# microsoft/M3P

Hardware: AMD Instinct MI355X
Metric: pre-train samples/sec (whole node), 12L/768d seq=128+36 (higher is better)
Workload: dtype bf16; 1 GPU; cfg2: 12L/768d/12h, 36 regions + 128 tokens, V=250002, 19 MLM targets/seq + ITM BCE, dropout 0.10, adam_inverse_sqrt + clip 5; per_gpu_batch=256, global_batch=256, seq_len=164, parallelism=dp1, prewarm_steps=36

## Files before the change

### m3p_amd/csrc/embed.hip

```cpp
#include "common.hpp"
#include <hip/amd_detail/amd_hip_unsafe_atomics.h>

namespace {

constexpr int EMB_BWD_BLOCKS = 512;

constexpr float kEps = 1e-12f;

template <int NI>
__device__ __forceinline__ void row_ln(const f32x4 (&v)[NI], int nchunk, int lane, float inv_d, float& mu, float& rs) {
  float s = 0.f;
#pragma unroll
  for (int i = 0; i < NI; ++i) s += (v[i][0] + v[i][1]) + (v[i][2] + v[i][3]);
  mu = wave_sum(s) * inv_d;
  float q = 0.f;
#pragma unroll
  for (int i = 0; i < NI; ++i) {
    if (lane + 64 * i < nchunk) {
      const f32x4 t = v[i] - mu;
      q += (t[0] * t[0] + t[1] * t[1]) + (t[2] * t[2] + t[3] * t[3]);
    }
  }
  rs = 1.0f / sqrtf(wave_sum(q) * inv_d + kEps);
}

struct EmbedFwdArgs {
  const int64_t* tok;
  const bf16* emb;
  const float* pos;
  const bf16* img_proj;
  const float* loc;
  const float* w_loc;
  const float* b_loc;
  const float* g_img; const float* be_img;
  const float* g_emb; const float* be_emb;
  const int32_t* totlen;
  bf16* h;
  bf16* z;
  float* mean_emb; float* rstd_emb;
  bf16* e;
  float* mean_img; float* rstd_img;
  int B, T, R, d;
  uint32_t seed_img, seed_emb, thresh24; float inv_keep;
  bf16* img_rows; int img_mode;
};

template <int NI>
__global__ __launch_bounds__(256) void embed_fwd_kernel(EmbedFwdArgs a) {
  const int lane = threadIdx.x & 63;
  const int wave = (blockIdx.x * blockDim.x + threadIdx.x) >> 6;
  const int nwaves = (gridDim.x * blockDim.x) >> 6;
  const int S = a.R + a.T, d = a.d, nchunk = d >> 2;
  const float inv_d = 1.0f / (float)d;
  for (int m = wave; m < a.B * S; m += nwaves) {
    const int b = m / S, s = m - b * S;
    const float mk = (a.img_mode == 1 || s < a.totlen[b]) ? 1.f : 0.f;
    f32x4 v[NI];
    if (s < a.R && a.img_mode == 2) {
#pragma unroll
      for (int i = 0; i < NI; ++i) {
        const int c = lane + 64 * i;
        v[i] = f32x4{0.f, 0.f, 0.f, 0.f};
        if (c < nchunk) v[i] = Vec4<bf16>::load(a.img_rows + ((size_t)b * a.R + s) * d + 4 * c);
      }
    } else if (s < a.R) {
      const int ri = s * a.B + b;
      float lc[5];
#pragma unroll
      for (int k = 0; k < 5; ++k) lc[k] = a.loc[(size_t)ri * 5 + k];
#pragma unroll
      for (int i = 0; i < NI; ++i) {
        const int c = lane + 64 * i;
        v[i] = f32x4{0.f, 0.f, 0.f, 0.f};
        if (c < nchunk) {
          f32x4 t = Vec4<bf16>::load(a.img_proj + (size_t)ri * d + 4 * c) + Vec4<float>::load(a.b_loc + 4 * c);
#pragma unroll
          for (int j = 0; j < 4; ++j) {
            const float* w = a.w_loc + (size_t)(4 * c + j) * 5;
            t[j] += w[0] * lc[0] + w[1] * lc[1] + w[2] * lc[2] + w[3] * lc[3] + w[4] * lc[4];
          }
          t = round_bf16(t);
          Vec4<bf16>::store(a.e + (size_t)ri * d + 4 * c, t);
          v[i] = t;
        }
      }
      float mu, rs;
      row_ln<NI>(v, nchunk, lane, inv_d, mu, rs);
      if (lane == 0) { a.mean_img[ri] = mu; a.rstd_img[ri] = rs; }
#pragma unroll
      for (int i = 0; i < NI; ++i) {
        const int c = lane + 64 * i;
        if (c < nchunk) {
          f32x4 o = (v[i] - mu) * rs * Vec4<float>::load(a.g_img + 4 * c) + Vec4<float>::load(a.be_img + 4 * c);
          if (a.thresh24) {
            const uint32_t base = (uint32_t)ri * (uint32_t)d + 4u * c;
            { bool kp[4]; m3p_keep_even<4>(base, a.seed_img, a.thresh24, kp);
#pragma unroll
          for (int j = 0; j < 4; ++j) o[j] = kp[j] ? o[j] * a.inv_keep : 0.f; }
          }
          v[i] = o;
          if (a.img_mode == 1) Vec4<bf16>::store(a.img_rows + ((size_t)b * a.R + s) * d + 4 * c, o);
        }
      }
      if (a.img_mode == 1) continue;
    } else {
      const int64_t id = a.tok[(size_t)(s - a.R) * a.B + b];
#pragma unroll
      for (int i = 0; i < NI; ++i) {
        const int c = lane + 64 * i;
        v[i] = f32x4{0.f, 0.f, 0.f, 0.f};
        if (c < nchunk) v[i] = Vec4<bf16>::load(a.emb + (size_t)id * d + 4 * c);
      }
    }
#pragma unroll
    for (int i = 0; i < NI; ++i) {
      const int c = lane + 64 * i;
      if (c < nchunk) {
        const f32x4 t = round_bf16((v[i] + Vec4<float>::load(a.pos + (size_t)s * d + 4 * c)) * mk);
        Vec4<bf16>::store(a.z + (size_t)m * d + 4 * c, t);
        v[i] = t;
      }
    }
    float mu, rs;
    row_ln<NI>(v, nchunk, lane, inv_d, mu, rs);
    if (lane == 0) { a.mean_emb[m] = mu; a.rstd_emb[m] = rs; }
#pragma unroll
    for (int i = 0; i < NI; ++i) {
      const int c = lane + 64 * i;
      if (c < nchunk) {
        f32x4 o = (v[i] - mu) * rs * Vec4<float>::load(a.g_emb + 4 * c) + Vec4<float>::load(a.be_emb + 4 * c);
        if (a.thresh24) {
          const uint32_t base = (uint32_t)m * (uint32_t)d + 4u * c;
          { bool kp[4]; m3p_keep_even<4>(base, a.seed_emb, a.thresh24, kp);
#pragma unroll
          for (int j = 0; j < 4; ++j) o[j] = kp[j] ? o[j] * a.inv_keep : 0.f; }
        }
        Vec4<bf16>::store(a.h + (size_t)m * d + 4 * c, o);
      }
    }
  }
}

struct EmbedBwdArgs {
  const bf16* dh;
  const bf16* z; const float* mean_emb; const float* rstd_emb; const float* g_emb;
  const bf16* e; const float* mean_img; const float* rstd_img; const float* g_img;
  const int64_t* tok; const int32_t* totlen; const float* loc;
  bf16* dz;
  bf16* de;
  float* d_g_emb; float* d_be_emb; float* d_pos;
  float* d_emb;
  bf16* d_tok_rows;
  float* d_g_img; float* d_be_img; float* d_b_img; float* d_b_loc; float* d_w_loc;
  int B, T, R, d, pad_index, bsplit;
  uint32_t seed_img, seed_emb, thresh24; float inv_keep;
};

template <int NI>
__device__ __forceinline__ void block_reduce_atomic(float (*red)[NI * 256], const f32x4 (&acc)[NI], float* out, int d,
                                                    int lane, int wib) {
#pragma unroll
  for (int i = 0; i < NI; ++i)
#pragma unroll
    for (int j = 0; j < 4; ++j) red[wib][4 * (lane + 64 * i) + j] = acc[i][j];
  __syncthreads();
  for (int c = threadIdx.x; c < d; c += blockDim.x)
    unsafeAtomicAdd(out + c, (red[0][c] + red[1][c]) + (red[2][c] + red[3][c]));
  __syncthreads();
}

template <int NI>
__global__ __launch_bounds__(256) void embed_bwd_rows_kernel(EmbedBwdArgs a) {
  __shared__ float red[4][NI * 256];
  const int lane = threadIdx.x & 63, wib = threadIdx.x >> 6;
  const int S = a.R + a.T, d = a.d, nchunk = d >> 2;
  const float inv_d = 1.0f / (float)d;
  const int s = blockIdx.x / a.bsplit, part = blockIdx.x - s * a.bsplit;
  f32x4 g[NI], acc_g[NI], acc_b[NI], acc_p[NI];
#pragma unroll
// ... 55 lines not shown
        if (c < nchunk) {
          f32x4 o = *reinterpret_cast<const f32x4*>(&red[wib][4 * c]);
          if (!live) o = f32x4{0.f, 0.f, 0.f, 0.f};
          Vec4<bf16>::store(dr + 4 * c, o);
        }
      }
    } else if (s >= a.R && id != a.pad_index && mk != 0.f) {
      float* de = a.d_emb + (size_t)id * d;
#pragma unroll
      for (int k = 0; k < 4 * NI; ++k) {
        const int e = lane + 64 * k;
        if (e < d) unsafeAtomicAdd(de + e, red[wib][e]);
      }
    }
  }
  __syncthreads();
  block_reduce_atomic<NI>(red, acc_g, a.d_g_emb, d, lane, wib);
  block_reduce_atomic<NI>(red, acc_b, a.d_be_emb, d, lane, wib);
  block_reduce_atomic<NI>(red, acc_p, a.d_pos + (size_t)s * d, d, lane, wib);
}

template <int NI>
__global__ __launch_bounds__(256) void embed_bwd_img_kernel(EmbedBwdArgs a) {
  __shared__ float red[4][NI * 256];
  const int lane = threadIdx.x & 63, wib = threadIdx.x >> 6;
  const int S = a.R + a.T, d = a.d, nchunk = d >> 2;
  const float inv_d = 1.0f / (float)d;
  const int r = blockIdx.x / a.bsplit, part = blockIdx.x - r * a.bsplit;
  f32x4 g[NI], acc_g[NI], acc_b[NI], acc_e[NI], acc_w[5][NI];
#pragma unroll
  for (int i = 0; i < NI; ++i) {
    const int c = lane + 64 * i;
    g[i] = f32x4{0.f, 0.f, 0.f, 0.f};
    if (c < nchunk) g[i] = Vec4<float>::load(a.g_img + 4 * c);
    acc_g[i] = acc_b[i] = acc_e[i] = f32x4{0.f, 0.f, 0.f, 0.f};
#pragma unroll
    for (int k = 0; k < 5; ++k) acc_w[k][i] = f32x4{0.f, 0.f, 0.f, 0.f};
  }
  for (int b = part * 4 + wib; b < a.B; b += 4 * a.bsplit) {
    const size_t m = (size_t)b * S + r;
    const size_t ri = (size_t)r * a.B + b;
    const float mu = a.mean_img[ri], rs = a.rstd_img[ri];
    float lc[5];
#pragma unroll
    for (int k = 0; k < 5; ++k) lc[k] = a.loc[ri * 5 + k];
    f32x4 dy[NI], xh[NI];
    float s1 = 0.f, s2 = 0.f;
#pragma unroll
    for (int i = 0; i < NI; ++i) {
      const int c = lane + 64 * i;
      dy[i] = xh[i] = f32x4{0.f, 0.f, 0.f, 0.f};
      if (c < nchunk) {
        dy[i] = Vec4<bf16>::load(a.dz + m * d + 4 * c);
        if (a.thresh24) {
          const uint32_t base = (uint32_t)ri * (uint32_t)d + 4u * c;
          { bool kp[4]; m3p_keep_even<4>(base, a.seed_img, a.thresh24, kp);
#pragma unroll
          for (int j = 0; j < 4; ++j) dy[i][j] = kp[j] ? dy[i][j] * a.inv_keep : 0.f; }
        }
        xh[i] = (Vec4<bf16>::load(a.e + ri * d + 4 * c) - mu) * rs;
        const f32x4 gd = dy[i] * g[i];
        s1 += (gd[0] + gd[1]) + (gd[2] + gd[3]);
        const f32x4 gx = gd * xh[i];
        s2 += (gx[0] + gx[1]) + (gx[2] + gx[3]);
        acc_g[i] += dy[i] * xh[i];
        acc_b[i] += dy[i];
      }
    }
    const float c1 = wave_sum(s1) * inv_d, c2 = wave_sum(s2) * inv_d;
#pragma unroll
    for (int i = 0; i < NI; ++i) {
      const int c = lane + 64 * i;
      if (c < nchunk) {
        const f32x4 ob = round_bf16((dy[i] * g[i] - c1 - xh[i] * c2) * rs);
        Vec4<bf16>::store(a.de + ri * d + 4 * c, ob);
        acc_e[i] += ob;
#pragma unroll
        for (int k = 0; k < 5; ++k) acc_w[k][i] += ob * lc[k];
      }
    }
  }
  block_reduce_atomic<NI>(red, acc_g, a.d_g_img, d, lane, wib);
  block_reduce_atomic<NI>(red, acc_b, a.d_be_img, d, lane, wib);
#pragma unroll
  for (int i = 0; i < NI; ++i)
#pragma unroll
    for (int j = 0; j < 4; ++j) red[wib][4 * (lane + 64 * i) + j] = acc_e[i][j];
  __syncthreads();
  for (int c = threadIdx.x; c < d; c += blockDim.x) {
    const float v = (red[0][c] + red[1][c]) + (red[2][c] + red[3][c]);
    unsafeAtomicAdd(a.d_b_img + c, v);
    unsafeAtomicAdd(a.d_b_loc + c, v);
  }
  __syncthreads();
#pragma unroll
  for (int k = 0; k < 5; ++k) {
#pragma unroll
    for (int i = 0; i < NI; ++i)
#pragma unroll
      for (int j = 0; j < 4; ++j) red[wib][4 * (lane + 64 * i) + j] = acc_w[k][i][j];
    __syncthreads();
    for (int c = threadIdx.x; c < d; c += blockDim.x)
      unsafeAtomicAdd(a.d_w_loc + (size_t)c * 5 + k, (red[0][c] + red[1][c]) + (red[2][c] + red[3][c]));
    __syncthreads();
  }
}

__global__ __launch_bounds__(256) void cast_f32_bf16_kernel(const float* __restrict__ src, bf16* __restrict__ dst, size_t n4) {
  for (size_t i = (size_t)blockIdx.x * blockDim.x + threadIdx.x; i < n4; i += (size_t)gridDim.x * blockDim.x)
    Vec4<bf16>::store(dst + 4 * i, Vec4<float>::load(src + 4 * i));
}

inline int ni_of(int d) { return (d + 255) / 256; }

int launch_embed_fwd(const EmbedFwdArgs& a, void* stream);
}

extern "C" {

int m3p_cast_f32_bf16(const float* src, void* dst, long long n, void* stream) {
  if (n <= 0 || (n % 4) != 0 || ((uintptr_t)src & 15) || ((uintptr_t)dst & 7)) return M3P_EINVAL;
  const size_t n4 = (size_t)n / 4;
  const int blocks = (int)((n4 + 255) / 256 < 4096 ? (n4 + 255) / 256 : 4096);
  hipLaunchKernelGGL(cast_f32_bf16_kernel, dim3(blocks), dim3(256), 0, (hipStream_t)stream, src, (bf16*)dst, n4);
  M3P_CHECK_LAUNCH();
  return M3P_OK;
}
// ... 9 lines not shown
  EmbedFwdArgs a = {tok, (const bf16*)emb_bf16, pos, (const bf16*)img_proj, loc, w_loc, b_loc, g_img, be_img, g_emb, be_emb,
                    totlen, (bf16*)h, (bf16*)z, mean_emb, rstd_emb, (bf16*)e, mean_img, rstd_img, B, T, R, d,
                    seed_img, seed_emb, thresh24, inv_keep, (bf16*)const_cast<void*>(img_rows), img_rows ? 2 : 0};
  return launch_embed_fwd(a, stream);
}

int m3p_embed_image_rows_fwd(const void* img_proj, const float* loc, const float* w_loc, const float* b_loc,
                             const float* g_img, const float* be_img, void* e, float* mean_img, float* rstd_img,
                             void* img_rows, int B, int R, int d, uint32_t seed_img, uint32_t thresh24, float inv_keep,
                             void* stream) {
  if (B <= 0 || R <= 0 || d <= 0 || (d % 4) != 0 || d > 1024 || !img_rows || ((uintptr_t)img_rows & 7)) return M3P_EINVAL;
  EmbedFwdArgs a = {nullptr, nullptr, nullptr, (const bf16*)img_proj, loc, w_loc, b_loc, g_img, be_img, nullptr, nullptr,
                    nullptr, nullptr, nullptr, nullptr, nullptr, (bf16*)e, mean_img, rstd_img, B, 0, R, d,
                    seed_img, 0u, thresh24, inv_keep, (bf16*)img_rows, 1};
  return launch_embed_fwd(a, stream);
}

}

namespace {
int launch_embed_fwd(const EmbedFwdArgs& a, void* stream) {
  const int B = a.B, T = a.T, R = a.R, d = a.d;
  const int rows = B * (R + T);
  const int blocks = (rows + 3) / 4 < 4096 ? (rows + 3) / 4 : 4096;
  hipStream_t st = (hipStream_t)stream;
  switch (ni_of(d)) {
    case 1: hipLaunchKernelGGL(embed_fwd_kernel<1>, dim3(blocks), dim3(256), 0, st, a); break;
    case 2: hipLaunchKernelGGL(embed_fwd_kernel<2>, dim3(blocks), dim3(256), 0, st, a); break;
    case 3: hipLaunchKernelGGL(embed_fwd_kernel<3>, dim3(blocks), dim3(256), 0, st, a); break;
    default: hipLaunchKernelGGL(embed_fwd_kernel<4>, dim3(blocks), dim3(256), 0, st, a); break;
  }
  M3P_CHECK_LAUNCH();
  return M3P_OK;
}
}

extern "C" {

int m3p_embed_assemble_bwd(const void* dh, const void* z, const float* mean_emb, const float* rstd_emb,
                           const float* g_emb, const void* e, const float* mean_img, const float* rstd_img,
                           const float* g_img, const int64_t* tok, const int32_t* totlen, const float* loc,
                           void* dz_scratch, void* de, float* d_g_emb, float* d_be_emb, float* d_pos, float* d_emb,
                           void* d_tok_rows, float* d_g_img, float* d_be_img, float* d_b_img, float* d_b_loc, float* d_w_loc,
                           int B, int T, int R, int d, int pad_index, uint32_t seed_img, uint32_t seed_emb,
                           uint32_t thresh24, float inv_keep, int phase, void* stream) {
  if (B <= 0 || T < 0 || R < 0 || d <= 0 || (d % 4) != 0 || d > 1024 || phase < 0 || phase > 2) return M3P_EINVAL;
  int bsplit = 1;
  while (bsplit < 16 && (R + T) * bsplit < EMB_BWD_BLOCKS && B / (4 * bsplit) >= 8) bsplit *= 2;
  EmbedBwdArgs a = {(const bf16*)dh, (const bf16*)z, mean_emb, rstd_emb, g_emb, (const bf16*)e, mean_img, rstd_img, g_img,
                    tok, totlen, loc, (bf16*)dz_scratch, (bf16*)de, d_g_emb, d_be_emb, d_pos, d_emb,
                    (bf16*)d_tok_rows, d_g_img, d_be_img, d_b_img, d_b_loc, d_w_loc, B, T, R, d, pad_index, bsplit,
                    seed_img, seed_emb, thresh24, inv_keep};
  hipStream_t st = (hipStream_t)stream;
  const int S = R + T;
#define M3P_EMB_BWD(NI)                                                                              \
  do {                                                                                               \
    if (phase != 2) hipLaunchKernelGGL(embed_bwd_rows_kernel<NI>, dim3(S* bsplit), dim3(256), 0, st, a);             \
    if (R > 0 && phase != 1) hipLaunchKernelGGL(embed_bwd_img_kernel<NI>, dim3(R* bsplit), dim3(256), 0, st, a);   \
  } while (0)
  switch (ni_of(d)) {
    case 1: M3P_EMB_BWD(1); break;
    case 2: M3P_EMB_BWD(2); break;
    case 3: M3P_EMB_BWD(3); break;
    default: M3P_EMB_BWD(4); break;
  }
#undef M3P_EMB_BWD
  M3P_CHECK_LAUNCH();
  return M3P_OK;
}

}
```

### m3p_amd/csrc/glue.hip

```cpp
#include "common.hpp"

namespace {

__global__ __launch_bounds__(256)
void seq_masks_kernel(const long long* __restrict__ len_a, const long long* __restrict__ len_b, int B, int S,
                      int* __restrict__ totlen, uint8_t* __restrict__ rowmask) {
  const int b = blockIdx.x;
  const int n = (int)(len_a[b] + (len_b ? len_b[b] : 0));
  if (threadIdx.x == 0) totlen[b] = n;
  for (int s = threadIdx.x; s < S; s += blockDim.x) rowmask[(size_t)b * S + s] = (s < n) ? 1 : 0;
}

__global__ __launch_bounds__(1024)
void mask_to_rows_kernel(const uint8_t* __restrict__ mask, int n_mask, int inner, long long s0, long long s1,
                         long long soff, int d, int* __restrict__ rows, int n_rows) {
  __shared__ int wsum[16];
  __shared__ int total_sh;
  const int tid = threadIdx.x, lane = tid & 63, w = tid >> 6;
  const int per = (n_mask + 1023) / 1024;
  const int lo = min(tid * per, n_mask), hi = min(lo + per, n_mask);
  int cnt = 0;
  for (int i = lo; i < hi; ++i) cnt += mask[i] ? 1 : 0;
  int inc = cnt;
#pragma unroll
  for (int o = 1; o < 64; o <<= 1) {
    const int v = __shfl_up(inc, o, 64);
    if (lane >= o) inc += v;
  }
  if (lane == 63) wsum[w] = inc;
  __syncthreads();
  if (tid == 0) {
    int run = 0;
    for (int i = 0; i < 16; ++i) { const int v = wsum[i]; wsum[i] = run; run += v; }
    total_sh = run;
  }
  __syncthreads();
  int pos = wsum[w] + inc - cnt;
  for (int i = lo; i < hi; ++i) {
    if (mask[i]) {
      if (pos < n_rows) {
        const int t = i / inner, b = i - t * inner;
        rows[pos] = (int)((soff + t * s0 + b * s1) / d);
      }
      ++pos;
    }
  }
  for (int k = total_sh + tid; k < n_rows; k += 1024) rows[k] = 0;
}

__global__ __launch_bounds__(256)
void cast_rows_kernel(const float* __restrict__ in, long long s0, long long s1, int n1, int cols,
                      bf16* __restrict__ out, long long nrows) {
  const int cpr = cols >> 2;
  const long long total = nrows * cpr;
  for (long long i = (long long)blockIdx.x * blockDim.x + threadIdx.x; i < total; i += (long long)gridDim.x * blockDim.x) {
    const long long row = i / cpr;
    const int c = (int)(i - row * cpr) * 4;
    const long long i0 = row / n1, i1 = row - i0 * n1;
    const f32x4 v = *reinterpret_cast<const f32x4*>(in + i0 * s0 + i1 * s1 + c);
    *reinterpret_cast<bf16x4*>(out + row * cols + c) = bf16x4{(bf16)v[0], (bf16)v[1], (bf16)v[2], (bf16)v[3]};
  }
}

template <typename TI>
__global__ __launch_bounds__(256)
void scale_to_bf16_kernel(const TI* __restrict__ in, const float* __restrict__ g, bf16* __restrict__ out, long long n4) {
  const float s = g[0];
  for (long long i = (long long)blockIdx.x * blockDim.x + threadIdx.x; i < n4; i += (long long)gridDim.x * blockDim.x) {
    f32x4 v = Vec4<TI>::load(in + 4 * i);
    v *= s;
    Vec4<bf16>::store(out + 4 * i, v);
  }
}

__global__ __launch_bounds__(256)
void axpy_dev_kernel(float* __restrict__ dst, const float* __restrict__ src, const float* __restrict__ g, long long n) {
  const float s = g[0];
  for (long long i = (long long)blockIdx.x * blockDim.x + threadIdx.x; i < n; i += (long long)gridDim.x * blockDim.x)
    dst[i] += s * src[i];
}

__device__ __forceinline__ float softplus_f(float x) {
  return fmaxf(x, 0.f) + log1pf(__expf(-fabsf(x)));
// ... 40 lines not shown

int grid_for(long long work, int per_block) {
  long long g = (work + per_block - 1) / per_block;
  return (int)(g < 1 ? 1 : (g > 2048 ? 2048 : g));
}

}

extern "C" {

int m3p_seq_masks(const int64_t* lengths, const int64_t* lengths_b, int B, int S, int32_t* totlen, uint8_t* rowmask,
                  void* stream) {
  if (B <= 0 || S <= 0 || !lengths || !totlen || !rowmask) return M3P_EINVAL;
  hipLaunchKernelGGL(seq_masks_kernel, dim3(B), dim3(256), 0, (hipStream_t)stream, (const long long*)lengths,
                     (const long long*)lengths_b, B, S, totlen, rowmask);
  M3P_CHECK_LAUNCH();
  return M3P_OK;
}

int m3p_mask_to_rows(const uint8_t* mask, int n_mask, int inner, long long s0, long long s1, long long soff, int d,
                     int32_t* rows, int n_rows, void* stream) {
  if (n_mask <= 0 || inner <= 0 || d <= 0 || n_rows < 0 || !mask || (n_rows && !rows)) return M3P_EINVAL;
  if (n_rows == 0) return M3P_OK;
  hipLaunchKernelGGL(mask_to_rows_kernel, dim3(1), dim3(1024), 0, (hipStream_t)stream, mask, n_mask, inner, s0, s1, soff, d,
                     rows, n_rows);
  M3P_CHECK_LAUNCH();
  return M3P_OK;
}

int m3p_cast_rows_f32_bf16(const float* in, long long s0, long long s1, int n0, int n1, int cols, void* out, void* stream) {
  if (n0 <= 0 || n1 <= 0 || cols <= 0 || (cols & 3) || (s0 & 3) || (s1 & 3) || ((uintptr_t)in & 15) || ((uintptr_t)out & 7))
    return M3P_EINVAL;
  const long long nrows = (long long)n0 * n1;
  hipLaunchKernelGGL(cast_rows_kernel, dim3(grid_for(nrows * (cols >> 2), 1024)), dim3(256), 0, (hipStream_t)stream, in, s0, s1,
                     n1, cols, (bf16*)out, nrows);
  M3P_CHECK_LAUNCH();
  return M3P_OK;
}

int m3p_scale_bf16_dev(const void* in, int in_is_f32, const float* g, void* out, long long n, void* stream) {
  if (n <= 0 || (n & 3) || !g || ((uintptr_t)in & (in_is_f32 ? 15 : 7)) || ((uintptr_t)out & 7)) return M3P_EINVAL;
  const int grid = grid_for(n >> 2, 1024);
  if (in_is_f32)
    hipLaunchKernelGGL(scale_to_bf16_kernel<float>, dim3(grid), dim3(256), 0, (hipStream_t)stream, (const float*)in, g, (bf16*)out, n >> 2);
  else
    hipLaunchKernelGGL(scale_to_bf16_kernel<bf16>, dim3(grid), dim3(256), 0, (hipStream_t)stream, (const bf16*)in, g, (bf16*)out, n >> 2);
  M3P_CHECK_LAUNCH();
  return M3P_OK;
}

int m3p_axpy_dev_f32(float* dst, const float* src, const float* g, long long n, void* stream) {
  if (n <= 0 || !dst || !src || !g) return M3P_EINVAL;
  hipLaunchKernelGGL(axpy_dev_kernel, dim3(grid_for(n, 1024)), dim3(256), 0, (hipStream_t)stream, dst, src, g, n);
  M3P_CHECK_LAUNCH();
  return M3P_OK;
}

int m3p_itm_loss_fwd_bwd(const float* scores, const int64_t* pos, int n_groups, int sample_n, float w_ce, float w_bce,
// ... 10 lines not shown
```

### m3p_amd/csrc/heads.hip

```cpp
#include "common.hpp"
#include <hip/amd_detail/amd_hip_unsafe_atomics.h>

namespace {

__global__ __launch_bounds__(256) void gather_rows_kernel(const bf16* __restrict__ src, const int32_t* __restrict__ idx,
                                                          bf16* __restrict__ dst, int n, int d) {
  const int nchunk = d >> 2;
  const size_t total = (size_t)n * nchunk;
  for (size_t i = (size_t)blockIdx.x * blockDim.x + threadIdx.x; i < total; i += (size_t)gridDim.x * blockDim.x) {
    const int r = (int)(i / nchunk), c = (int)(i - (size_t)r * nchunk);
    *reinterpret_cast<bf16x4*>(dst + (size_t)r * d + 4 * c) =
        *reinterpret_cast<const bf16x4*>(src + (size_t)idx[r] * d + 4 * c);
  }
}
__global__ __launch_bounds__(256) void place_rows_kernel(const bf16* __restrict__ src, const int32_t* __restrict__ inv,
                                                         bf16* __restrict__ dst, int rows, int d, int n, uint32_t fill2) {
  typedef unsigned int u32x4 __attribute__((ext_vector_type(4)));
  const int nchunk = d >> 3;
  const size_t total = (size_t)rows * nchunk;
  const u32x4 fv = u32x4{fill2, fill2, fill2, fill2};
  for (size_t i = (size_t)blockIdx.x * blockDim.x + threadIdx.x; i < total; i += (size_t)gridDim.x * blockDim.x) {
    const int r = (int)(i / nchunk), c = (int)(i - (size_t)r * nchunk);
    const int j = inv[r];
    u32x4 v = fv;
// ... 209 lines not shown
      lb[u] = row_lse[r] * kLog2e;
      tc[u] = (int)(target[r] - col0);
    }
#pragma unroll
    for (int u = 0; u < U; ++u) {
      if (rb + u < r1) {
        bf16x8 g;
#pragma unroll
        for (int j = 0; j < 8; ++j) {
          float q = (col0 + j < V) ? __builtin_amdgcn_exp2f(__builtin_fmaf((float)v[u][j], kLog2e, -lb[u])) : 0.f;
          if (j == tc[u]) q -= 1.f;
          g[j] = (bf16)(q * gscale);
          cs[j] += (float)g[j];
        }
        *reinterpret_cast<bf16x8*>(logits + (size_t)(rb + u) * ld + col0) = g;
      }
    }
  }
  float* out = part + (size_t)blockIdx.y * ld + col0;
  *reinterpret_cast<f32x4*>(out) = f32x4{cs[0], cs[1], cs[2], cs[3]};
  *reinterpret_cast<f32x4*>(out + 4) = f32x4{cs[4], cs[5], cs[6], cs[7]};
}

__global__ __launch_bounds__(256) void ce_colsum_reduce_kernel(const float* __restrict__ part, int ld, int n_groups, float* __restrict__ out) {
  const int c = (blockIdx.x * 256 + threadIdx.x) * 4;
  if (c >= ld) return;
  const int per = (n_groups + gridDim.y - 1) / gridDim.y;
  const int g0 = blockIdx.y * per, g1 = min(n_groups, g0 + per);
  f32x4 acc = {0.f, 0.f, 0.f, 0.f};
  for (int g = g0; g < g1; ++g) acc += *reinterpret_cast<const f32x4*>(part + (size_t)g * ld + c);
#pragma unroll
  for (int j = 0; j < 4; ++j) unsafeAtomicAdd(out + c + j, acc[j]);
}

__global__ __launch_bounds__(256) void colsum_kernel(const bf16* __restrict__ x, int ld, int n, int ncols,
                                                     float* __restrict__ out, const float* __restrict__ scale_ptr) {
  const int c4 = blockIdx.x * blockDim.x + threadIdx.x;
  if (4 * c4 >= ncols) return;
  const int rows_per = (n + gridDim.y - 1) / gridDim.y;
  const int r0 = blockIdx.y * rows_per, r1 = min(n, r0 + rows_per);
  f32x4 acc = {0.f, 0.f, 0.f, 0.f};
  for (int r = r0; r < r1; ++r) acc += Vec4<bf16>::load(x + (size_t)r * ld + 4 * c4);
  const float sc = scale_ptr ? *scale_ptr : 1.f;
#pragma unroll
  for (int j = 0; j < 4; ++j)
    if (4 * c4 + j < ncols) unsafeAtomicAdd(out + 4 * c4 + j, acc[j] * sc);
}

}

extern "C" {

size_t m3p_ce_colsum_workspace_bytes(int ld, int n_rows) {
  return (size_t)((n_rows + CE_RB - 1) / CE_RB) * (size_t)ld * sizeof(float);
}
// ... 107 lines not shown
```

### m3p_amd/csrc/itm.hip

```cpp
#include "common.hpp"

namespace {

__global__ __launch_bounds__(256) void itm_score_fwd_kernel(const bf16* __restrict__ pre, const float* __restrict__ w2,
                                                            const float* __restrict__ b2, float* __restrict__ pooled,
                                                            float* __restrict__ scores, int d) {
  __shared__ float red[4];
  const int b = blockIdx.x, tid = threadIdx.x, lane = tid & 63, wid = tid >> 6;
  float s = 0.f;
  for (int j = tid; j < d; j += 256) {
    const float p = tanhf((float)pre[(size_t)b * d + j]);
    pooled[(size_t)b * d + j] = p;
    s += w2[j] * p;
  }
  s = wave_sum(s);
  if (lane == 0) red[wid] = s;
  __syncthreads();
  if (tid == 0) scores[b] = red[0] + red[1] + red[2] + red[3] + b2[0];
}

__global__ __launch_bounds__(256) void itm_score_bwd_rows_kernel(const float* __restrict__ dscores, const float* __restrict__ pooled,
                                                                 const float* __restrict__ w2, bf16* __restrict__ dpre16,
                                                                 bf16* __restrict__ dpreT16, int ldt, int d) {
  const int b = blockIdx.x;
  const float ds = dscores[b];
  for (int j = threadIdx.x; j < d; j += 256) {
    const float p = pooled[(size_t)b * d + j];
    const bf16 g = (bf16)(ds * w2[j] * (1.f - p * p));
    dpre16[(size_t)b * d + j] = g;
    dpreT16[(size_t)j * ldt + b] = g;
  }
}

__global__ __launch_bounds__(256) void itm_score_bwd_cols_kernel(const float* __restrict__ dscores, const float* __restrict__ pooled,
                                                                 const float* __restrict__ w2, float* __restrict__ db1,
                                                                 float* __restrict__ dw2, float* __restrict__ db2, int B, int d) {
  __shared__ float s1[4][64], s2[4][64], s3[4];
  const int jl = threadIdx.x & 63, bg = threadIdx.x >> 6;
  const int j = blockIdx.x * 64 + jl;
  float a1 = 0.f, a2 = 0.f, a3 = 0.f;
  if (j < d) {
    const float w = w2[j];
    for (int b = bg; b < B; b += 4) {
      const float ds = dscores[b], p = pooled[(size_t)b * d + j];
      a1 += ds * w * (1.f - p * p);
      a2 += ds * p;
      if (jl == 0) a3 += ds;
    }
  }
  s1[bg][jl] = a1; s2[bg][jl] = a2;
  if (jl == 0) s3[bg] = a3;
  __syncthreads();
  if (bg == 0 && j < d) {
    db1[j] += (s1[0][jl] + s1[1][jl]) + (s1[2][jl] + s1[3][jl]);
    dw2[j] += (s2[0][jl] + s2[1][jl]) + (s2[2][jl] + s2[3][jl]);
  }
  if (blockIdx.x == 0 && threadIdx.x == 0) db2[0] += (s3[0] + s3[1]) + (s3[2] + s3[3]);
}

}

extern "C" {

int m3p_itm_score_fwd(const void* pre, const float* w2, const float* b2, float* pooled, float* scores, int B, int d,
                      void* stream) {
  if (B <= 0 || d <= 0) return M3P_EINVAL;
  hipLaunchKernelGGL(itm_score_fwd_kernel, dim3(B), dim3(256), 0, (hipStream_t)stream, (const bf16*)pre, w2, b2, pooled,
                     scores, d);
  M3P_CHECK_LAUNCH();
  return M3P_OK;
}

int m3p_itm_score_bwd(const float* dscores, const float* pooled, const float* w2, void* dpre16, void* dpreT16, int ldt,
                      float* db1, float* dw2, float* db2, int B, int d, void* stream) {
  if (B <= 0 || d <= 0 || ldt < B) return M3P_EINVAL;
  hipLaunchKernelGGL(itm_score_bwd_rows_kernel, dim3(B), dim3(256), 0, (hipStream_t)stream, dscores, pooled, w2,
                     (bf16*)dpre16, (bf16*)dpreT16, ldt, d);
  M3P_CHECK_LAUNCH();
  hipLaunchKernelGGL(itm_score_bwd_cols_kernel, dim3((d + 63) / 64), dim3(256), 0, (hipStream_t)stream, dscores, pooled, w2,
                     db1, dw2, db2, B, d);
  M3P_CHECK_LAUNCH();
  return M3P_OK;
}

}
```

Baseline: 7847 sequences/s.

## Prefetch rows in embedding kernels and vectorize small glue reduction kernels

The embedding forward and image-backward kernels now issue the next row's loads before computing the current row (software prefetch), and the forward kernel stages w_loc transposed in LDS. Image-backward reductions are folded in two shared-memory stages with their own block split. Separately, mask_to_rows counts bits with 16-byte vector loads, cast_rows gains an 8-wide nontemporal path, the CE column-sum reduce is unrolled with coalesced atomics, and the ITM column kernel uses 1024 threads. These target memory latency and launch inefficiency in small kernels, at the cost of extra registers and LDS per block.

```diff
diff --git a/m3p_amd/csrc/embed.hip b/m3p_amd/csrc/embed.hip
--- a/m3p_amd/csrc/embed.hip
+++ b/m3p_amd/csrc/embed.hip
@@ -4,6 +4,8 @@
 namespace {
 
 constexpr int EMB_BWD_BLOCKS = 512;
+constexpr int EMB_BWD_IMG_BLOCKS = 256;
+constexpr int EMB_FWD_BLOCKS = 1536;
 
 constexpr float kEps = 1e-12f;
 
@@ -46,39 +48,83 @@
 };
 
 template <int NI>
+struct FwdRow {
+  bf16x4 raw[NI];
+  float lc[5];
+  int tl;
+};
+
+__device__ __forceinline__ int64_t embed_fwd_token(const EmbedFwdArgs& a, int m) {
+  const int S = a.R + a.T, b = m / S, s = m - b * S;
+  return s >= a.R ? a.tok[(size_t)(s - a.R) * a.B + b] : 0;
+}
+
+template <int NI>
+__device__ __forceinline__ void embed_fwd_request(const EmbedFwdArgs& a, int m, int64_t id, int lane, FwdRow<NI>& r) {
+  const int S = a.R + a.T, d = a.d, nchunk = d >> 2;
+  const int b = m / S, s = m - b * S;
+  r.tl = a.img_mode == 1 ? 0 : a.totlen[b];
+  const bf16* src;
+  if (s >= a.R) {
+    src = a.emb + (size_t)id * d;
+  } else if (a.img_mode == 2) {
+    src = a.img_rows + ((size_t)b * a.R + s) * d;
+  } else {
+    const int ri = s * a.B + b;
+    src = a.img_proj + (size_t)ri * d;
+#pragma unroll
+    for (int k = 0; k < 5; ++k) r.lc[k] = a.loc[(size_t)ri * 5 + k];
+  }
+#pragma unroll
+  for (int i = 0; i < NI; ++i) {
+    const int c = lane + 64 * i;
+    r.raw[i] = bf16x4{(bf16)0.f, (bf16)0.f, (bf16)0.f, (bf16)0.f};
+    if (c < nchunk) r.raw[i] = *reinterpret_cast<const bf16x4*>(src + 4 * c);
+  }
+}
+
+__device__ __forceinline__ f32x4 widen(bf16x4 v) { return f32x4{(float)v[0], (float)v[1], (float)v[2], (float)v[3]}; }
+
+template <int NI>
 __global__ __launch_bounds__(256) void embed_fwd_kernel(EmbedFwdArgs a) {
+  __shared__ __attribute__((aligned(16))) float wl[5][NI * 256];
   const int lane = threadIdx.x & 63;
   const int wave = (blockIdx.x * blockDim.x + threadIdx.x) >> 6;
   const int nwaves = (gridDim.x * blockDim.x) >> 6;
-  const int S = a.R + a.T, d = a.d, nchunk = d >> 2;
+  const int S = a.R + a.T, d = a.d, nchunk = d >> 2, rows = a.B * S;
   const float inv_d = 1.0f / (float)d;
-  for (int m = wave; m < a.B * S; m += nwaves) {
+  if (a.R > 0 && a.img_mode != 2) {
+    for (int i = threadIdx.x; i < 5 * d; i += 256) {
+      const int c = i / 5;
+      wl[i - 5 * c][c] = a.w_loc[i];
+    }
+    __syncthreads();
+  }
+  if (wave >= rows) return;
+  FwdRow<NI> nx;
+  embed_fwd_request<NI>(a, wave, embed_fwd_token(a, wave), lane, nx);
+  int64_t idn = wave + nwaves < rows ? embed_fwd_token(a, wave + nwaves) : 0;
+  for (int m = wave; m < rows; m += nwaves) {
     const int b = m / S, s = m - b * S;
-    const float mk = (a.img_mode == 1 || s < a.totlen[b]) ? 1.f : 0.f;
+    const FwdRow<NI> cu = nx;
+    if (m + nwaves < rows) {
+      embed_fwd_request<NI>(a, m + nwaves, idn, lane, nx);
+      if (m + 2 * nwaves < rows) idn = embed_fwd_token(a, m + 2 * nwaves);
+    }
+    const float mk = (a.img_mode == 1 || s < cu.tl) ? 1.f : 0.f;
     f32x4 v[NI];
-    if (s < a.R && a.img_mode == 2) {
+#pragma unroll
+    for (int i = 0; i < NI; ++i) v[i] = widen(cu.raw[i]);
+    if (s < a.R && a.img_mode != 2) {
+      const int ri = s * a.B + b;
 #pragma unroll
       for (int i = 0; i < NI; ++i) {
         const int c = lane + 64 * i;
-        v[i] = f32x4{0.f, 0.f, 0.f, 0.f};
-        if (c < nchunk) v[i] = Vec4<bf16>::load(a.img_rows + ((size_t)b * a.R + s) * d + 4 * c);
-      }
-    } else if (s < a.R) {
-      const int ri = s * a.B + b;
-      float lc[5];
-#pragma unroll
-      for (int k = 0; k < 5; ++k) lc[k] = a.loc[(size_t)ri * 5 + k];
-#pragma unroll
-      for (int i = 0; i < NI; ++i) {
-        const int c = lane + 64 * i;
-        v[i] = f32x4{0.f, 0.f, 0.f, 0.f};
         if (c < nchunk) {
-          f32x4 t = Vec4<bf16>::load(a.img_proj + (size_t)ri * d + 4 * c) + Vec4<float>::load(a.b_loc + 4 * c);
-#pragma unroll
-          for (int j = 0; j < 4; ++j) {
-            const float* w = a.w_loc + (size_t)(4 * c + j) * 5;
-            t[j] += w[0] * lc[0] + w[1] * lc[1] + w[2] * lc[2] + w[3] * lc[3] + w[4] * lc[4];
-          }
+          f32x4 t = v[i] + Vec4<float>::load(a.b_loc + 4 * c);
+          t += Vec4<float>::load(&wl[0][4 * c]) * cu.lc[0] + Vec4<float>::load(&wl[1][4 * c]) * cu.lc[1] +
+               Vec4<float>::load(&wl[2][4 * c]) * cu.lc[2] + Vec4<float>::load(&wl[3][4 * c]) * cu.lc[3] +
+               Vec4<float>::load(&wl[4][4 * c]) * cu.lc[4];
           t = round_bf16(t);
           Vec4<bf16>::store(a.e + (size_t)ri * d + 4 * c, t);
           v[i] = t;
@@ -103,14 +149,6 @@
         }
       }
       if (a.img_mode == 1) continue;
-    } else {
-      const int64_t id = a.tok[(size_t)(s - a.R) * a.B + b];
-#pragma unroll
-      for (int i = 0; i < NI; ++i) {
-        const int c = lane + 64 * i;
-        v[i] = f32x4{0.f, 0.f, 0.f, 0.f};
-        if (c < nchunk) v[i] = Vec4<bf16>::load(a.emb + (size_t)id * d + 4 * c);
-      }
     }
 #pragma unroll
     for (int i = 0; i < NI; ++i) {
@@ -152,9 +190,37 @@
   float* d_emb;
   bf16* d_tok_rows;
   float* d_g_img; float* d_be_img; float* d_b_img; float* d_b_loc; float* d_w_loc;
-  int B, T, R, d, pad_index, bsplit;
+  int B, T, R, d, pad_index, bsplit, bsplit_img;
   uint32_t seed_img, seed_emb, thresh24; float inv_keep;
 };
+
+template <int NI>
+__device__ __forceinline__ float* fold_at(float* red, int half, int q, int nq) { return red + (size_t)(half * nq + q) * (NI * 256); }
+
+template <int NI, int NQ>
+__device__ __forceinline__ void block_fold(float* red, f32x4 (&acc)[NQ][NI], int lane, int wib) {
+  if (wib >= 2) {
+#pragma unroll
+    for (int q = 0; q < NQ; ++q)
+#pragma unroll
+      for (int i = 0; i < NI; ++i) Vec4<float>::store(fold_at<NI>(red, wib - 2, q, NQ) + 4 * (lane + 64 * i), acc[q][i]);
+  }
+  __syncthreads();
+  if (wib < 2) {
+#pragma unroll
+    for (int q = 0; q < NQ; ++q)
+#pragma unroll
+      for (int i = 0; i < NI; ++i) acc[q][i] += Vec4<float>::load(fold_at<NI>(red, wib, q, NQ) + 4 * (lane + 64 * i));
+  }
+  __syncthreads();
+  if (wib < 2) {
+#pragma unroll
+    for (int q = 0; q < NQ; ++q)
+#pragma unroll
+      for (int i = 0; i < NI; ++i) Vec4<float>::store(fold_at<NI>(red, wib, q, NQ) + 4 * (lane + 64 * i), acc[q][i]);
+  }
+  __syncthreads();
+}
 
 template <int NI>
 __device__ __forceinline__ void block_reduce_atomic(float (*red)[NI * 256], const f32x4 (&acc)[NI], float* out, int d,
@@ -256,28 +322,44 @@
 
 template <int NI>
 __global__ __launch_bounds__(256) void embed_bwd_img_kernel(EmbedBwdArgs a) {
-  __shared__ float red[4][NI * 256];
+  __shared__ __attribute__((aligned(16))) float red[10 * NI * 256];
   const int lane = threadIdx.x & 63, wib = threadIdx.x >> 6;
   const int S = a.R + a.T, d = a.d, nchunk = d >> 2;
   const float inv_d = 1.0f / (float)d;
-  const int r = blockIdx.x / a.bsplit, part = blockIdx.x - r * a.bsplit;
-  f32x4 g[NI], acc_g[NI], acc_b[NI], acc_e[NI], acc_w[5][NI];
+  const int r = blockIdx.x / a.bsplit_img, part = blockIdx.x - r * a.bsplit_img;
+  f32x4 g[NI], acc[3][NI], acc_w[5][NI];
 #pragma unroll
   for (int i = 0; i < NI; ++i) {
     const int c = lane + 64 * i;
     g[i] = f32x4{0.f, 0.f, 0.f, 0.f};
     if (c < nchunk) g[i] = Vec4<float>::load(a.g_img + 4 * c);
-    acc_g[i] = acc_b[i] = acc_e[i] = f32x4{0.f, 0.f, 0.f, 0.f};
+    acc[0][i] = acc[1][i] = acc[2][i] = f32x4{0.f, 0.f, 0.f, 0.f};
 #pragma unroll
     for (int k = 0; k < 5; ++k) acc_w[k][i] = f32x4{0.f, 0.f, 0.f, 0.f};
   }
-  for (int b = part * 4 + wib; b < a.B; b += 4 * a.bsplit) {
+  struct Req { bf16x4 dz[NI], e[NI]; float mu, rs, lc[5]; } nx;
+  auto request = [&](int b, Req& q) {
     const size_t m = (size_t)b * S + r;
     const size_t ri = (size_t)r * a.B + b;
-    const float mu = a.mean_img[ri], rs = a.rstd_img[ri];
-    float lc[5];
-#pragma unroll
-    for (int k = 0; k < 5; ++k) lc[k] = a.loc[ri * 5 + k];
+    q.mu = a.mean_img[ri]; q.rs = a.rstd_img[ri];
+#pragma unroll
+    for (int k = 0; k < 5; ++k) q.lc[k] = a.loc[ri * 5 + k];
+#pragma unroll
+    for (int i = 0; i < NI; ++i) {
+      const int c = lane + 64 * i;
+      if (c < nchunk) {
+        q.dz[i] = *reinterpret_cast<const bf16x4*>(a.dz + m * d + 4 * c);
+        q.e[i] = *reinterpret_cast<const bf16x4*>(a.e + ri * d + 4 * c);
+      }
+    }
+  };
+  const int b0 = part * 4 + wib, bstep = 4 * a.bsplit_img;
+  if (b0 < a.B) request(b0, nx);
+  for (int b = b0; b < a.B; b += bstep) {
+    const size_t ri = (size_t)r * a.B + b;
+    const Req cu = nx;
+    if (b + bstep < a.B) request(b + bstep, nx);
+    const float mu = cu.mu, rs = cu.rs;
     f32x4 dy[NI], xh[NI];
     float s1 = 0.f, s2 = 0.f;
 #pragma unroll
@@ -285,20 +367,20 @@
       const int c = lane + 64 * i;
       dy[i] = xh[i] = f32x4{0.f, 0.f, 0.f, 0.f};
       if (c < nchunk) {
-        dy[i] = Vec4<bf16>::load(a.dz + m * d + 4 * c);
+        dy[i] = widen(cu.dz[i]);
         if (a.thresh24) {
           const uint32_t base = (uint32_t)ri * (uint32_t)d + 4u * c;
           { bool kp[4]; m3p_keep_even<4>(base, a.seed_img, a.thresh24, kp);
 #pragma unroll
           for (int j = 0; j < 4; ++j) dy[i][j] = kp[j] ? dy[i][j] * a.inv_keep : 0.f; }
         }
-        xh[i] = (Vec4<bf16>::load(a.e + ri * d + 4 * c) - mu) * rs;
+        xh[i] = (widen(cu.e[i]) - mu) * rs;
         const f32x4 gd = dy[i] * g[i];
         s1 += (gd[0] + gd[1]) + (gd[2] + gd[3]);
         const f32x4 gx = gd * xh[i];
         s2 += (gx[0] + gx[1]) + (gx[2] + gx[3]);
-        acc_g[i] += dy[i] * xh[i];
-        acc_b[i] += dy[i];
+        acc[0][i] += dy[i] * xh[i];
+        acc[1][i] += dy[i];
       }
     }
     const float c1 = wave_sum(s1) * inv_d, c2 = wave_sum(s2) * inv_d;
@@ -308,35 +390,25 @@
       if (c < nchunk) {
         const f32x4 ob = round_bf16((dy[i] * g[i] - c1 - xh[i] * c2) * rs);
         Vec4<bf16>::store(a.de + ri * d + 4 * c, ob);
-        acc_e[i] += ob;
-#pragma unroll
-        for (int k = 0; k < 5; ++k) acc_w[k][i] += ob * lc[k];
-      }
-    }
-  }
-  block_reduce_atomic<NI>(red, acc_g, a.d_g_img, d, lane, wib);
-  block_reduce_atomic<NI>(red, acc_b, a.d_be_img, d, lane, wib);
-#pragma unroll
-  for (int i = 0; i < NI; ++i)
-#pragma unroll
-    for (int j = 0; j < 4; ++j) red[wib][4 * (lane + 64 * i) + j] = acc_e[i][j];
-  __syncthreads();
+        acc[2][i] += ob;
+#pragma unroll
+        for (int k = 0; k < 5; ++k) acc_w[k][i] += ob * cu.lc[k];
+      }
+    }
+  }
+  block_fold<NI, 3>(red, acc, lane, wib);
   for (int c = threadIdx.x; c < d; c += blockDim.x) {
-    const float v = (red[0][c] + red[1][c]) + (red[2][c] + red[3][c]);
+    unsafeAtomicAdd(a.d_g_img + c, fold_at<NI>(red, 0, 0, 3)[c] + fold_at<NI>(red, 1, 0, 3)[c]);
+    unsafeAtomicAdd(a.d_be_img + c, fold_at<NI>(red, 0, 1, 3)[c] + fold_at<NI>(red, 1, 1, 3)[c]);
+    const float v = fold_at<NI>(red, 0, 2, 3)[c] + fold_at<NI>(red, 1, 2, 3)[c];
     unsafeAtomicAdd(a.d_b_img + c, v);
     unsafeAtomicAdd(a.d_b_loc + c, v);
   }
   __syncthreads();
-#pragma unroll
-  for (int k = 0; k < 5; ++k) {
-#pragma unroll
-    for (int i = 0; i < NI; ++i)
-#pragma unroll
-      for (int j = 0; j < 4; ++j) red[wib][4 * (lane + 64 * i) + j] = acc_w[k][i][j];
-    __syncthreads();
-    for (int c = threadIdx.x; c < d; c += blockDim.x)
-      unsafeAtomicAdd(a.d_w_loc + (size_t)c * 5 + k, (red[0][c] + red[1][c]) + (red[2][c] + red[3][c]));
-    __syncthreads();
+  block_fold<NI, 5>(red, acc_w, lane, wib);
+  for (int i = threadIdx.x; i < 5 * d; i += blockDim.x) {
+    const int c = i / 5, k = i - 5 * c;
+    unsafeAtomicAdd(a.d_w_loc + i, fold_at<NI>(red, 0, k, 5)[c] + fold_at<NI>(red, 1, k, 5)[c]);
   }
 }
 
@@ -392,7 +464,7 @@
 int launch_embed_fwd(const EmbedFwdArgs& a, void* stream) {
   const int B = a.B, T = a.T, R = a.R, d = a.d;
   const int rows = B * (R + T);
-  const int blocks = (rows + 3) / 4 < 4096 ? (rows + 3) / 4 : 4096;
+  const int blocks = (rows + 3) / 4 < EMB_FWD_BLOCKS ? (rows + 3) / 4 : EMB_FWD_BLOCKS;
   hipStream_t st = (hipStream_t)stream;
   switch (ni_of(d)) {
     case 1: hipLaunchKernelGGL(embed_fwd_kernel<1>, dim3(blocks), dim3(256), 0, st, a); break;
@@ -417,16 +489,18 @@
   if (B <= 0 || T < 0 || R < 0 || d <= 0 || (d % 4) != 0 || d > 1024 || phase < 0 || phase > 2) return M3P_EINVAL;
   int bsplit = 1;
   while (bsplit < 16 && (R + T) * bsplit < EMB_BWD_BLOCKS && B / (4 * bsplit) >= 8) bsplit *= 2;
+  int bsplit_img = 1;
+  while (bsplit_img < 16 && R * bsplit_img < EMB_BWD_IMG_BLOCKS && B / (4 * bsplit_img) >= 4) bsplit_img *= 2;
   EmbedBwdArgs a = {(const bf16*)dh, (const bf16*)z, mean_emb, rstd_emb, g_emb, (const bf16*)e, mean_img, rstd_img, g_img,
                     tok, totlen, loc, (bf16*)dz_scratch, (bf16*)de, d_g_emb, d_be_emb, d_pos, d_emb,
                     (bf16*)d_tok_rows, d_g_img, d_be_img, d_b_img, d_b_loc, d_w_loc, B, T, R, d, pad_index, bsplit,
-                    seed_img, seed_emb, thresh24, inv_keep};
+                    bsplit_img, seed_img, seed_emb, thresh24, inv_keep};
   hipStream_t st = (hipStream_t)stream;
   const int S = R + T;
 #define M3P_EMB_BWD(NI)                                                                              \
   do {                                                                                               \
     if (phase != 2) hipLaunchKernelGGL(embed_bwd_rows_kernel<NI>, dim3(S* bsplit), dim3(256), 0, st, a);             \
-    if (R > 0 && phase != 1) hipLaunchKernelGGL(embed_bwd_img_kernel<NI>, dim3(R* bsplit), dim3(256), 0, st, a);   \
+    if (R > 0 && phase != 1) hipLaunchKernelGGL(embed_bwd_img_kernel<NI>, dim3(R* bsplit_img), dim3(256), 0, st, a); \
   } while (0)
   switch (ni_of(d)) {
     case 1: M3P_EMB_BWD(1); break;
diff --git a/m3p_amd/csrc/glue.hip b/m3p_amd/csrc/glue.hip
--- a/m3p_amd/csrc/glue.hip
+++ b/m3p_amd/csrc/glue.hip
@@ -11,16 +11,41 @@
   for (int s = threadIdx.x; s < S; s += blockDim.x) rowmask[(size_t)b * S + s] = (s < n) ? 1 : 0;
 }
 
+__device__ __forceinline__ uint32_t nz_bytes(uint32_t w) {
+  return (((w & 0x7f7f7f7fu) + 0x7f7f7f7fu) | w) & 0x80808080u;
+}
+typedef __attribute__((ext_vector_type(4))) uint32_t u32x4;
+
+__device__ __forceinline__ u32x4 mask_piece(const uint8_t* __restrict__ base, int v0, int vlo, int vhi) {
+  u32x4 w;
+  if (v0 >= vlo && v0 + 16 <= vhi) {
+    w = *reinterpret_cast<const u32x4*>(base + v0);
+  } else {
+    w = u32x4{0u, 0u, 0u, 0u};
+    for (int j = 0; j < 16; ++j)
+      if (v0 + j >= vlo && v0 + j < vhi && base[v0 + j]) w[j >> 2] |= 1u << (8 * (j & 3));
+  }
+  return u32x4{nz_bytes(w[0]), nz_bytes(w[1]), nz_bytes(w[2]), nz_bytes(w[3])};
+}
+
+template <bool WIDE>
 __global__ __launch_bounds__(1024)
 void mask_to_rows_kernel(const uint8_t* __restrict__ mask, int n_mask, int inner, long long s0, long long s1,
                          long long soff, int d, int* __restrict__ rows, int n_rows) {
   __shared__ int wsum[16];
   __shared__ int total_sh;
   const int tid = threadIdx.x, lane = tid & 63, w = tid >> 6;
-  const int per = (n_mask + 1023) / 1024;
-  const int lo = min(tid * per, n_mask), hi = min(lo + per, n_mask);
+  const int off = (int)((uintptr_t)mask & 15);
+  const uint8_t* base = mask - off;
+  const int vlo = off, vhi = off + n_mask;
+  const int per = ((vhi + 1023) / 1024 + 15) & ~15;
+  const int lo = min(tid * per, vhi), hi = min(lo + per, vhi);
   int cnt = 0;
-  for (int i = lo; i < hi; ++i) cnt += mask[i] ? 1 : 0;
+#pragma unroll 4
+  for (int v0 = lo; v0 < hi; v0 += 16) {
+    const u32x4 m = mask_piece(base, v0, vlo, vhi);
+    cnt += (__popc(m[0]) + __popc(m[1])) + (__popc(m[2]) + __popc(m[3]));
+  }
   int inc = cnt;
 #pragma unroll
   for (int o = 1; o < 64; o <<= 1) {
@@ -36,13 +61,24 @@
   }
   __syncthreads();
   int pos = wsum[w] + inc - cnt;
-  for (int i = lo; i < hi; ++i) {
-    if (mask[i]) {
-      if (pos < n_rows) {
-        const int t = i / inner, b = i - t * inner;
-        rows[pos] = (int)((soff + t * s0 + b * s1) / d);
+  if (cnt) {
+    for (int v0 = lo; v0 < hi; v0 += 16) {
+      const u32x4 m = mask_piece(base, v0, vlo, vhi);
+#pragma unroll
+      for (int q = 0; q < 4; ++q) {
+        uint32_t bits = m[q];
+        while (bits) {
+          const int j = (__ffs(bits) - 1) >> 3;
+          bits &= bits - 1;
+          if (pos < n_rows) {
+            const int i = v0 + 4 * q + j - off;
+            const uint32_t t = (uint32_t)i / (uint32_t)inner, b = (uint32_t)i - t * (uint32_t)inner;
+            if (WIDE) rows[pos] = (int)((soff + (long long)t * s0 + (long long)b * s1) / d);
+            else rows[pos] = (int)(((uint32_t)soff + t * (uint32_t)s0 + b * (uint32_t)s1) / (uint32_t)d);
+          }
+          ++pos;
+        }
       }
-      ++pos;
     }
   }
   for (int k = total_sh + tid; k < n_rows; k += 1024) rows[k] = 0;
@@ -59,6 +95,37 @@
     const long long i0 = row / n1, i1 = row - i0 * n1;
     const f32x4 v = *reinterpret_cast<const f32x4*>(in + i0 * s0 + i1 * s1 + c);
     *reinterpret_cast<bf16x4*>(out + row * cols + c) = bf16x4{(bf16)v[0], (bf16)v[1], (bf16)v[2], (bf16)v[3]};
+  }
+}
+
+__global__ __launch_bounds__(256)
+void cast_rows8_kernel(const float* __restrict__ in, long long s0, long long s1, int n1, int cols,
+                       bf16* __restrict__ out, long long nrows) {
+  const int cpr = cols >> 3;
+  const long long total = nrows * cpr, stride = (long long)gridDim.x * blockDim.x;
+  auto src = [&](long long i) {
+    const long long row = i / cpr;
+    const int c = (int)(i - row * cpr) * 8;
+    const long long i0 = row / n1, i1 = row - i0 * n1;
+    return in + i0 * s0 + i1 * s1 + c;
+  };
+  auto ld = [](const float* p) { return __builtin_nontemporal_load(reinterpret_cast<const f32x4*>(p)); };
+  auto put = [&](long long i, f32x4 a, f32x4 b) {
+    const bf16x8 o = bf16x8{(bf16)a[0], (bf16)a[1], (bf16)a[2], (bf16)a[3], (bf16)b[0], (bf16)b[1], (bf16)b[2], (bf16)b[3]};
+    __builtin_nontemporal_store(o, reinterpret_cast<bf16x8*>(out + i * 8));
+  };
+  for (long long i = (long long)blockIdx.x * blockDim.x + threadIdx.x; i < total; i += 2 * stride) {
+    const long long i2 = i + stride;
+    const float* p = src(i);
+    const f32x4 a0 = ld(p), a1 = ld(p + 4);
+    if (i2 < total) {
+      const float* q = src(i2);
+      const f32x4 b0 = ld(q), b1 = ld(q + 4);
+      put(i, a0, a1);
+      put(i2, b0, b1);
+    } else {
+      put(i, a0, a1);
+    }
   }
 }
 
@@ -145,8 +212,15 @@
                      int32_t* rows, int n_rows, void* stream) {
   if (n_mask <= 0 || inner <= 0 || d <= 0 || n_rows < 0 || !mask || (n_rows && !rows)) return M3P_EINVAL;
   if (n_rows == 0) return M3P_OK;
-  hipLaunchKernelGGL(mask_to_rows_kernel, dim3(1), dim3(1024), 0, (hipStream_t)stream, mask, n_mask, inner, s0, s1, soff, d,
-                     rows, n_rows);
+  const long long tmax = (n_mask - 1) / inner, bmax = inner - 1;
+  const bool narrow = s0 >= 0 && s1 >= 0 && soff >= 0 && s0 <= 0x7fffffff && s1 <= 0x7fffffff &&
+                      soff + tmax * s0 + bmax * s1 <= 0x7fffffff;
+  if (narrow)
+    hipLaunchKernelGGL(mask_to_rows_kernel<false>, dim3(1), dim3(1024), 0, (hipStream_t)stream, mask, n_mask, inner, s0, s1, soff,
+                       d, rows, n_rows);
+  else
+    hipLaunchKernelGGL(mask_to_rows_kernel<true>, dim3(1), dim3(1024), 0, (hipStream_t)stream, mask, n_mask, inner, s0, s1, soff,
+                       d, rows, n_rows);
   M3P_CHECK_LAUNCH();
   return M3P_OK;
 }
@@ -155,8 +229,12 @@
   if (n0 <= 0 || n1 <= 0 || cols <= 0 || (cols & 3) || (s0 & 3) || (s1 & 3) || ((uintptr_t)in & 15) || ((uintptr_t)out & 7))
     return M3P_EINVAL;
   const long long nrows = (long long)n0 * n1;
-  hipLaunchKernelGGL(cast_rows_kernel, dim3(grid_for(nrows * (cols >> 2), 1024)), dim3(256), 0, (hipStream_t)stream, in, s0, s1,
-                     n1, cols, (bf16*)out, nrows);
+  if ((cols & 7) == 0 && ((uintptr_t)out & 15) == 0)
+    hipLaunchKernelGGL(cast_rows8_kernel, dim3(grid_for(nrows * (cols >> 3), 512)), dim3(256), 0, (hipStream_t)stream, in, s0, s1,
+                       n1, cols, (bf16*)out, nrows);
+  else
+    hipLaunchKernelGGL(cast_rows_kernel, dim3(grid_for(nrows * (cols >> 2), 1024)), dim3(256), 0, (hipStream_t)stream, in, s0, s1,
+                       n1, cols, (bf16*)out, nrows);
   M3P_CHECK_LAUNCH();
   return M3P_OK;
 }
diff --git a/m3p_amd/csrc/heads.hip b/m3p_amd/csrc/heads.hip
--- a/m3p_amd/csrc/heads.hip
+++ b/m3p_amd/csrc/heads.hip
@@ -255,15 +255,34 @@
   *reinterpret_cast<f32x4*>(out + 4) = f32x4{cs[4], cs[5], cs[6], cs[7]};
 }
 
+__device__ __forceinline__ f32x4 ld_once(const float* p) { return __builtin_nontemporal_load(reinterpret_cast<const f32x4*>(p)); }
+
 __global__ __launch_bounds__(256) void ce_colsum_reduce_kernel(const float* __restrict__ part, int ld, int n_groups, float* __restrict__ out) {
+  __shared__ __attribute__((aligned(16))) float tr[4][256];
+  const int lane = threadIdx.x & 63, wib = threadIdx.x >> 6;
   const int c = (blockIdx.x * 256 + threadIdx.x) * 4;
-  if (c >= ld) return;
   const int per = (n_groups + gridDim.y - 1) / gridDim.y;
   const int g0 = blockIdx.y * per, g1 = min(n_groups, g0 + per);
   f32x4 acc = {0.f, 0.f, 0.f, 0.f};
-  for (int g = g0; g < g1; ++g) acc += *reinterpret_cast<const f32x4*>(part + (size_t)g * ld + c);
-#pragma unroll
-  for (int j = 0; j < 4; ++j) unsafeAtomicAdd(out + c + j, acc[j]);
+  if (c < ld) {
+    const float* p = part + c;
+    int g = g0;
+    for (; g + 4 <= g1; g += 4) {
+      const f32x4 v0 = ld_once(p + (size_t)g * ld);
+      const f32x4 v1 = ld_once(p + (size_t)(g + 1) * ld);
+      const f32x4 v2 = ld_once(p + (size_t)(g + 2) * ld);
+      const f32x4 v3 = ld_once(p + (size_t)(g + 3) * ld);
+      acc += (v0 + v1) + (v2 + v3);
+    }
+    for (; g < g1; ++g) acc += ld_once(p + (size_t)g * ld);
+  }
+  *reinterpret_cast<f32x4*>(&tr[wib][4 * lane]) = acc;
+  const int cw = (blockIdx.x * 256 + wib * 64) * 4;
+#pragma unroll
+  for (int k = 0; k < 4; ++k) {
+    const int e = lane + 64 * k;
+    if (cw + e < ld) unsafeAtomicAdd(out + cw + e, tr[wib][e]);
+  }
 }
 
 __global__ __launch_bounds__(256) void colsum_kernel(const bf16* __restrict__ x, int ld, int n, int ncols,
diff --git a/m3p_amd/csrc/itm.hip b/m3p_amd/csrc/itm.hip
--- a/m3p_amd/csrc/itm.hip
+++ b/m3p_amd/csrc/itm.hip
@@ -32,30 +32,50 @@
   }
 }
 
-__global__ __launch_bounds__(256) void itm_score_bwd_cols_kernel(const float* __restrict__ dscores, const float* __restrict__ pooled,
-                                                                 const float* __restrict__ w2, float* __restrict__ db1,
-                                                                 float* __restrict__ dw2, float* __restrict__ db2, int B, int d) {
-  __shared__ float s1[4][64], s2[4][64], s3[4];
+constexpr int ITM_BG = 16;
+__global__ __launch_bounds__(1024) void itm_score_bwd_cols_kernel(const float* __restrict__ dscores, const float* __restrict__ pooled,
+                                                                  const float* __restrict__ w2, float* __restrict__ db1,
+                                                                  float* __restrict__ dw2, float* __restrict__ db2, int B, int d) {
+  __shared__ float s1[ITM_BG][64], s2[ITM_BG][64], s3[ITM_BG];
   const int jl = threadIdx.x & 63, bg = threadIdx.x >> 6;
   const int j = blockIdx.x * 64 + jl;
   float a1 = 0.f, a2 = 0.f, a3 = 0.f;
   if (j < d) {
     const float w = w2[j];
-    for (int b = bg; b < B; b += 4) {
+    int b = bg;
+    for (; b + 3 * ITM_BG < B; b += 4 * ITM_BG) {
+      float ds[4], p[4];
+#pragma unroll
+      for (int u = 0; u < 4; ++u) { ds[u] = dscores[b + u * ITM_BG]; p[u] = pooled[(size_t)(b + u * ITM_BG) * d + j]; }
+#pragma unroll
+      for (int u = 0; u < 4; ++u) {
+        a1 += ds[u] * w * (1.f - p[u] * p[u]);
+        a2 += ds[u] * p[u];
+        a3 += ds[u];
+      }
+    }
+    for (; b < B; b += ITM_BG) {
       const float ds = dscores[b], p = pooled[(size_t)b * d + j];
       a1 += ds * w * (1.f - p * p);
       a2 += ds * p;
-      if (jl == 0) a3 += ds;
+      a3 += ds;
     }
   }
   s1[bg][jl] = a1; s2[bg][jl] = a2;
   if (jl == 0) s3[bg] = a3;
   __syncthreads();
   if (bg == 0 && j < d) {
-    db1[j] += (s1[0][jl] + s1[1][jl]) + (s1[2][jl] + s1[3][jl]);
-    dw2[j] += (s2[0][jl] + s2[1][jl]) + (s2[2][jl] + s2[3][jl]);
+    float t1 = 0.f, t2 = 0.f;
+#pragma unroll
+    for (int u = 0; u < ITM_BG; ++u) { t1 += s1[u][jl]; t2 += s2[u][jl]; }
+    db1[j] += t1;
+    dw2[j] += t2;
   }
-  if (blockIdx.x == 0 && threadIdx.x == 0) db2[0] += (s3[0] + s3[1]) + (s3[2] + s3[3]);
+  if (blockIdx.x == 0 && threadIdx.x == 0) {
+    float t3 = 0.f;
+    for (int u = 0; u < ITM_BG; ++u) t3 += s3[u];
+    db2[0] += t3;
+  }
 }
 
 }
@@ -77,7 +97,7 @@
   hipLaunchKernelGGL(itm_score_bwd_rows_kernel, dim3(B), dim3(256), 0, (hipStream_t)stream, dscores, pooled, w2,
                      (bf16*)dpre16, (bf16*)dpreT16, ldt, d);
   M3P_CHECK_LAUNCH();
-  hipLaunchKernelGGL(itm_score_bwd_cols_kernel, dim3((d + 63) / 64), dim3(256), 0, (hipStream_t)stream, dscores, pooled, w2,
+  hipLaunchKernelGGL(itm_score_bwd_cols_kernel, dim3((d + 63) / 64), dim3(1024), 0, (hipStream_t)stream, dscores, pooled, w2,
                      db1, dw2, db2, B, d);
   M3P_CHECK_LAUNCH();
   return M3P_OK;
```

Result: no change. 7868 sequences/s, median of 6 (+0.3%).
